# fkluger/vanishing_points_2017

Measured on AMD Instinct MI355X. Metric: images/sec (LSD->CNN->EM) + horizon-AUC parity, YUD-shape, 1/2/4/8 GPU, higher is better.
Workload: dtype f32 (CNN: f32 operands / accumulation / results; conv1 multiply EXACT bf16 pieces of the f32 operands (three per operand) on the bf16 matrix cores; conv2-5, fc6 and fc7 multiply scaled fp16 PAIRS of the f32 operands (22 of 24 significand bits, three exact products per f32 product) on the fp16 matrix

## Files before the change

### __graft_entry__.py

```python
import os
import subprocess
import sys

ROOT = os.path.dirname(os.path.abspath(__file__))
if ROOT not in sys.path:
    sys.path.insert(0, ROOT)


def build():
    from vanishing_points_2017_amd import build as vbuild
    so = vbuild.build(verbose=True)
    sim = os.path.join(ROOT, "tests", "hostsim")
    out = os.path.join(sim, "_build")
    os.makedirs(out, exist_ok=True)
    subprocess.check_call(["g++", "-O2", "-std=c++17", "-ffp-contract=off", "-fPIC", "-shared",
                           "-Wno-unknown-pragmas", os.path.join(sim, "sim_em.cpp"), "-o",
                           os.path.join(out, "libvpk_hostsim.so")])
    subprocess.check_call(["g++", "-O2", "-std=c++17", "-ffp-contract=off", "-fPIC", "-shared",
                           os.path.join(sim, "sim_raster.cpp"), "-o", os.path.join(out, "libvpk_hostsim_raster.so")])
    subprocess.check_call(["g++", "-O2", "-std=c++17", "-Wall", "-Werror", "-fPIC", "-shared",
                           os.path.join(sim, "sim_cnn_plan.cpp"), "-o", os.path.join(out, "libvpk_hostsim_cnn_plan.so")])
    odir = os.path.join(ROOT, "oracle", "_build")
    os.makedirs(odir, exist_ok=True)
    subprocess.check_call(["gcc", "-O2", "-fPIC", "-shared", "-ffp-contract=off", "-fno-builtin",
                           os.path.join(ROOT, "oracle", "_fma.c"), "-o", os.path.join(odir, "libvpkfma.so"), "-lm"])
    import vanishing_points_2017_amd
    from vanishing_points_2017_amd import _lib
    lib = _lib.load()
    missing = [s for s in _lib.EXPORTS if not hasattr(lib, s)]
    if missing:
        raise RuntimeError("libvpk.so lacks symbols: %s" % missing)
    print("built", so)


def smoke():
    import numpy as np
    import torch
    assert torch.cuda.is_available(), "smoke() needs cuda:0"
    from vanishing_points_2017_amd import synth, vp_localisation
    from oracle import em_numpy
    from oracle import agg_raster
    from vanishing_points_2017_amd import sphere_mapping
    sc = synth.make_scene(4242, 90, 3)
    ln = sc["l"]
    sc["sphere_image"] = sphere_mapping.sphere_line_plot(ln.copy(), 500, alpha=0.1)
    assert np.array_equal(sc["sphere_image"], agg_raster.raster(ln)), "the sphere raster differs from the oracle"
    got = vp_localisation.expectation_maximisation(sc["l"].copy(), sc["lp"].copy(), sc["cnn_response"],
                                                   sphere_image=sc["sphere_image"])
    ref = em_numpy.expectation_maximisation(sc["l"].copy(), sc["lp"].copy(), sc["cnn_response"].copy(),
                                            sphere_image=sc["sphere_image"])
    assert np.array_equal(got["vp_assoc"], ref["vp_assoc"]), "line->VP assignments differ from the oracle"
    assert np.abs(got["vp"] - ref["vp"]).max() < 1e-4
    from oracle import cnn_torch
    from vanishing_points_2017_amd import cnn
    w, mean = cnn.synthetic_weights(0), cnn.synthetic_mean(0)
    sphere = sc["sphere_image"][None]
    want = cnn_torch.forward(w, mean, sphere)
    net = cnn.Net(w, mean)
    err = []
    for alg in (4, 2):
        net.set_algorithm(alg)
        err.append(float(np.abs(net.forward(sphere) - want).max()))
    net.set_algorithm(4)
    assert max(err) <= 2e-5, "CNN response differs from the oracle: %s" % err
    print("smoke ok: raster of %d lines exact; %d VPs, %d iterations; CNN max |diff| %.1e (default: fp16 pairs) / %.1e (exact bf16 triples + Winograd f32)" % (
        ln.shape[0], got["vp"].shape[0], got["iterations"], err[0], err[1]))


if __name__ == "__main__":
    build()
    if len(sys.argv) > 1 and sys.argv[1] == "smoke":
        smoke()
```

### vanishing_points_2017_amd/csrc/cnn_dense_pieces.hpp

```cpp
#ifndef VPK_CNN_DENSE_PIECES_HPP_
#define VPK_CNN_DENSE_PIECES_HPP_

namespace {

constexpr int DP_THREADS = 512;
constexpr int DP_BM = 256, DP_BN = 128;
constexpr int DP_CHUNK = 32;
template <int NP> constexpr int DP_STAGE = NP * 2 * 4 * 1024;
constexpr int DP_NST = 3;
constexpr int DP_FOLD = 8;

struct DenseDims {
    int N, K, OC;
    int chunks, kparts, cpp;
    int mtiles, ntiles;
    float wscale, oscale;
    const int* live = nullptr;
};

template <int NP>
__global__ __launch_bounds__(256) void dense_split_kernel(const float* __restrict__ x, unsigned short* __restrict__ out, int N, int K,
                                                          int chunks, float ascale, unsigned* __restrict__ range_word, unsigned range_bit,
                                                          unsigned* __restrict__ img_range, const int* __restrict__ live) {
    const int c = blockIdx.x, nt = blockIdx.y;
    if (live) {
        N = __builtin_amdgcn_readfirstlane(*live);
        if (nt * DP_BN >= N) return;
    }
    const int j = threadIdx.x >> 6, lane = threadIdx.x & 63;
    const int n = nt * DP_BN + 32 * j + (lane & 31), h = lane >> 5;
    float v[16];
    if (n < N) {
        const f32x4v* src = reinterpret_cast<const f32x4v*>(x + (size_t)n * K + (size_t)c * DP_CHUNK + 16 * h);
#pragma unroll
        for (int q = 0; q < 4; ++q) {
            const f32x4v t = src[q];
            v[4 * q] = t[0]; v[4 * q + 1] = t[1]; v[4 * q + 2] = t[2]; v[4 * q + 3] = t[3];
        }
    } else {
#pragma unroll
        for (int e = 0; e < 16; ++e) v[e] = 0.f;
    }
    unsigned short p[3][16];
    bool bad = false;
#pragma unroll
    for (int e = 0; e < 16; ++e) {
        if (NP == 3) split3(v[e], p[0][e], p[1][e], p[2][e]);
        else split2h_guard(v[e] * ascale, p[0][e], p[1][e], bad);
    }
    if (NP == 2) {
        const unsigned long long m = __builtin_amdgcn_ballot_w64(bad);
        if (m != 0ull) {
            if (lane == 0) atomicOr(range_word, range_bit);
            if (img_range && lane < 32 && (((m | (m >> 32)) >> lane) & 1ull)) atomicOr(img_range + n, range_bit);
        }
    }
    u32x4* dst = reinterpret_cast<u32x4*>(out + ((size_t)nt * chunks + c) * (DP_STAGE<NP> / 2));
#pragma unroll
    for (int q = 0; q < NP; ++q)
#pragma unroll
        for (int s = 0; s < 2; ++s) {
            u32x4 w4;
#pragma unroll
            for (int e = 0; e < 4; ++e) w4[e] = (unsigned)p[q][8 * s + 2 * e] | ((unsigned)p[q][8 * s + 2 * e + 1] << 16);
            dst[(((q * 2 + s) * 4 + j) * 64) + lane] = w4;
        }
}

__global__ void dense_tile_weights_kernel(const float* __restrict__ w, float* __restrict__ out, int OC, int K, int chunks, long long total4) {
    const long long o4 = (long long)blockIdx.x * blockDim.x + threadIdx.x;
    if (o4 >= total4) return;
    const int kk4 = (int)(o4 % (DP_CHUNK / 4));
    const int r = (int)((o4 / (DP_CHUNK / 4)) % DP_BM);
    const long long tc = o4 / ((DP_CHUNK / 4) * DP_BM);
    const int c = (int)(tc % chunks);
    const int mt = (int)(tc / chunks);
    const int row = mt * DP_BM + r;
    f32x4v v = {0.f, 0.f, 0.f, 0.f};
    if (row < OC) v = *reinterpret_cast<const f32x4v*>(w + (size_t)row * K + (size_t)c * DP_CHUNK + 4 * kk4);
    reinterpret_cast<f32x4v*>(out)[o4] = v;
}

__global__ void dense_pair_weights_kernel(const float* __restrict__ w, unsigned short* __restrict__ out, int OC, int K, int chunks,
                                          float wscale, long long total16) {
    const long long o = (long long)blockIdx.x * blockDim.x + threadIdx.x;
    if (o >= total16) return;
    const int lane = (int)(o & 63);
    const int q = (int)((o >> 6) & 1), s_ = (int)((o >> 7) & 1), wv = (int)((o >> 8) & 7);
    const long long tc = o >> 11;
    const int c = (int)(tc % chunks), mt = (int)(tc / chunks);
    const int row = mt * DP_BM + 32 * wv + (lane & 31), h = lane >> 5;
    unsigned short p[8];
#pragma unroll
    for (int e = 0; e < 8; ++e) {
        const float x = row < OC ? w[(size_t)row * K + (size_t)c * DP_CHUNK + 16 * h + 8 * s_ + e] * wscale : 0.f;
        unsigned short h0, h1;
        split2h(x, h0, h1);
        p[e] = q == 0 ? h0 : h1;
    }
    u32x4 w4;
#pragma unroll
    for (int e = 0; e < 4; ++e) w4[e] = (unsigned)p[2 * e] | ((unsigned)p[2 * e + 1] << 16);
    reinterpret_cast<u32x4*>(out)[o] = w4;
}

__global__ __launch_bounds__(DP_THREADS, 2) void dense_pairs_kernel(DenseDims d, const unsigned short* __restrict__ wpair,
                                                                    const unsigned short* __restrict__ xfrag, float* __restrict__ part,
                                                                    int* __restrict__ item_counter, int total_items) {
    constexpr int NP = 2;
    __shared__ __attribute__((aligned(16))) unsigned char dp_lds[DP_NST * DP_STAGE<NP>];
    __shared__ int s_next[2];
    const int tid = threadIdx.x, lane = tid & 63;
    const int wave = __builtin_amdgcn_readfirstlane(tid >> 6);
    const int r31 = lane & 31, h = lane >> 5;
    const unsigned lds0 = lds_addr(dp_lds);
    typedef __attribute__((address_space(3))) const bf16x8 lds_cbf8;
    int parity = 0;
    for (int item = blockIdx.x; item < total_items;) {
        int nx = 0;
// ... 227 lines not shown
```

### vanishing_points_2017_amd/csrc/cnn_plan.hpp

```cpp
#ifndef VPK_CNN_PLAN_HPP_
#define VPK_CNN_PLAN_HPP_

#include "../../include/vpk.h"

struct CnnConfig {
    int precision = 0;
    int split_variant = 0;
    int algorithm = 4;
    int fusion = 3;
    int conv1_group = 4;
    int dense_presplit = 1;
    bool profiling = false;
};

inline void cnn_config_set_precision(CnnConfig& c, int mode) {
    c.precision = mode ? 1 : 0;
    c.split_variant = mode > 1 ? mode - 1 : 0;
}

enum class Conv1Impl { GEMM, DIRECT_F32, GEMM_FUSED, PIECES3, PIECES2 };
enum class ConvImpl { DMA_F32, SPLIT_GEMM, WINOGRAD, PIECES3, PIECES2 };
enum class DenseImpl { DMA_F32, PIECES3, PIECES2_STREAMED, PIECES2_PRESPLIT };

struct ConvStage {
    ConvImpl impl = ConvImpl::DMA_F32;
    int split_tiling = 0;
    bool chained_in = false;
    bool chained_out = false;
    bool needs_to_planes = false;
    bool writes_next_planes = false;
};

struct CnnPlan {
    int err = VPK_OK;
    const char* msg = nullptr;
    bool prep_input = false;
    Conv1Impl conv1 = Conv1Impl::PIECES3;
    bool conv1_hands_planes = false;
    ConvStage conv[4];
    bool norm2_planes = false;
    bool norm2_hands_planes = false;
    DenseImpl fc[3] = {DenseImpl::DMA_F32, DenseImpl::DMA_F32, DenseImpl::DMA_F32};
};

inline CnnPlan cnn_resolve_plan(const CnnConfig& c, int tap, bool f32_images, bool device_counted) {
    CnnPlan p;
    const bool f32_mfma = c.precision == 0;
    const bool pairs = f32_mfma && c.algorithm == 4;
    const bool triples = f32_mfma && c.algorithm >= 2 && !pairs;
    const bool wino = f32_mfma && c.algorithm >= 1;
    const bool split = c.precision == 1;

    if (tap == 0 || c.fusion == 0) p.conv1 = Conv1Impl::GEMM;
    else if (c.fusion == 1) p.conv1 = Conv1Impl::DIRECT_F32;
    else if (c.fusion == 2) p.conv1 = Conv1Impl::GEMM_FUSED;
    else p.conv1 = c.fusion == 4 ? Conv1Impl::PIECES2 : Conv1Impl::PIECES3;
    p.prep_input = p.conv1 == Conv1Impl::GEMM || p.conv1 == Conv1Impl::GEMM_FUSED;
    const bool conv1_pieces = p.conv1 == Conv1Impl::PIECES3 || p.conv1 == Conv1Impl::PIECES2;
    p.conv1_hands_planes = conv1_pieces && pairs && tap != 1;
    if (f32_images && p.conv1 == Conv1Impl::PIECES2) {
        p.err = VPK_ERR_STATE;
        p.msg = "vpk_cnn_forward_f32: vpk_cnn_set_fusion(4) takes uint8 rasters only";
    }

    const ConvImpl pieces = pairs ? ConvImpl::PIECES2 : ConvImpl::PIECES3;
    const ConvImpl other = split ? ConvImpl::SPLIT_GEMM : (wino ? ConvImpl::WINOGRAD : ConvImpl::DMA_F32);
    const bool pieces35 = pairs || (triples && c.algorithm == 3);
    p.conv[0].impl = pairs || triples ? pieces : other;
    p.conv[1].impl = pieces35 ? pieces : other;
    p.conv[2].impl = pairs ? pieces : other;
    p.conv[3].impl = pieces35 ? pieces : other;
    p.norm2_planes = pairs;
    p.norm2_hands_planes = pairs && tap != 3;
    p.conv[1].writes_next_planes = pairs && tap != 4;
    p.conv[2].writes_next_planes = pairs && tap != 5;
    p.conv[0].needs_to_planes = (pairs || triples) && !p.conv1_hands_planes;
    p.conv[1].needs_to_planes = pieces35 && !p.norm2_hands_planes;
    p.conv[2].needs_to_planes = pairs && !p.conv[1].writes_next_planes;
    p.conv[3].needs_to_planes = pieces35 && !p.conv[2].writes_next_planes;
    const bool chain = split && tap != 4 && tap != 5;
    p.conv[1].chained_out = p.conv[2].chained_in = p.conv[2].chained_out = p.conv[3].chained_in = chain;
    for (int i = 0; i < 4; ++i) p.conv[i].split_tiling = c.split_variant == 0 ? (i <= 1 ? 1 : 0) : c.split_variant - 1;

    const DenseImpl dense2 = c.dense_presplit ? DenseImpl::PIECES2_PRESPLIT : DenseImpl::PIECES2_STREAMED;
    if (pairs) p.fc[0] = p.fc[1] = dense2;
    else if (triples) p.fc[0] = DenseImpl::PIECES3;

    if (device_counted) {
        const bool counted = p.conv1 == Conv1Impl::PIECES3 && p.conv[0].impl == ConvImpl::PIECES3 &&
                             p.conv[1].impl == ConvImpl::WINOGRAD && p.conv[2].impl == ConvImpl::WINOGRAD &&
                             p.conv[3].impl == ConvImpl::WINOGRAD && !p.norm2_planes && p.fc[0] == DenseImpl::PIECES3 &&
                             p.fc[1] == DenseImpl::DMA_F32 && p.fc[2] == DenseImpl::DMA_F32 && tap < 0 && !c.profiling;
        if (!counted) {
            p.err = VPK_ERR_STATE;
            p.msg = "run_forward: a device-counted pass runs algorithm 2 with the default conv1, untapped";
        }
    }
    return p;
}

#endif
```

### vanishing_points_2017_amd/csrc/cnn_topology.hpp

```cpp
#ifndef VPK_CNN_TOPOLOGY_HPP_
#define VPK_CNN_TOPOLOGY_HPP_

#include <stddef.h>

namespace {

struct Topo { int IC, H, W, OC, OH, OW, G, KH, S, P, BM, OP; };
constexpr Topo TOPO[8] = {
    {1, 500, 500, 96, 123, 123, 1, 11, 4, 0, 96, 0},
    {48, 61, 61, 128, 61, 61, 2, 5, 1, 2, 128, 0},
    {256, 30, 30, 384, 30, 30, 1, 3, 1, 1, 128, 1},
    {192, 30, 30, 192, 30, 30, 2, 3, 1, 1, 96, 1},
    {192, 30, 30, 128, 30, 30, 2, 3, 1, 1, 128, 0},
    {57600, 1, 1, 4096, 1, 1, 1, 1, 1, 0, 128, 0},
    {4096, 1, 1, 4096, 1, 1, 1, 1, 1, 0, 128, 0},
    {4096, 1, 1, 400, 1, 1, 1, 1, 1, 0, 128, 0},
};
constexpr int KSPLIT[8] = {1, 1, 1, 1, 1, 72, 16, 32};
constexpr size_t splitk_partials_per_image() {
    size_t m = 0;
    for (int li = 5; li < 8; ++li) m = (size_t)KSPLIT[li] * TOPO[li].OC > m ? (size_t)KSPLIT[li] * TOPO[li].OC : m;
    return m;
}

enum Region { R_IN, R_CONV1, R_POOL1, R_CONV2, R_POOL2, R_CONV3, R_CONV4, R_CONV5, R_POOL5, R_FCA, R_FCB, R_PART, R_SPLIT, R_SPLIT4, R_SPLIT5, R_P6_2, R_P6_3, R_P6_5, R_COUNT };
constexpr int MAX_CHUNK = 4096;
constexpr size_t CTR_FLOATS = 64;
constexpr size_t GUARD_FLOATS = 64;
static_assert(GUARD_FLOATS * sizeof(float) >= 8 * 16, "the patch DMA's overrun: 8 words of 16 bytes");
constexpr size_t REGION_FLOATS[R_COUNT] = {
    500ull * 500,
    96ull * 123 * 123,
    96ull * 65 * 65,
    256ull * 61 * 61,
    256ull * 32 * 32,
    384ull * 32 * 32,
    384ull * 32 * 32,
    256ull * 900,
    256ull * 225,
    4096, 4096,
    splitk_partials_per_image(),
    96ull * 65 * 65 * 3 / 2,
    384ull * 32 * 32 * 3 / 2,
    384ull * 32 * 32 * 3 / 2,
    96ull * 65 * 65 * 3 / 2,
    256ull * 32 * 32 * 3 / 2,
    384ull * 32 * 32 * 3 / 2,
};
constexpr size_t arena_floats_per_image() {
    size_t t = 0;
    for (int i = 0; i < R_COUNT; ++i) t += REGION_FLOATS[i];
    return t;
}
constexpr size_t A_CONV1 = 96ull * 123 * 123, A_POOL1 = 96ull * 61 * 61;
constexpr size_t A_CONV2 = 256ull * 61 * 61, A_POOL2 = 256ull * 30 * 30;
constexpr size_t A_CONV3 = 384ull * 900, A_CONV4 = 384ull * 900, A_CONV5 = 256ull * 900, A_POOL5 = 256ull * 225;
constexpr size_t A_FC6 = 4096, A_FC7 = 4096, A_FC8 = 400;

}
#endif
```

### vanishing_points_2017_amd/csrc/vpk_cnn.hip

```cpp
#include "vpk_internal.hpp"

#include <stdlib.h>
#include <string.h>
#include <type_traits>
#include <vector>

#include "cnn_plan.hpp"
#include "cnn_topology.hpp"
#include "cnn_gemm_f32.hpp"
#include "cnn_conv1_direct.hpp"
#include "cnn_norm_pool.hpp"

namespace {

#include "cnn_split_gemm.hpp"
#include "cnn_pairs.hpp"
#include "cnn_conv1_pieces.hpp"
#include "cnn_conv_pieces.hpp"
#include "cnn_norm_pool_planes.hpp"
#include "cnn_dense_pieces.hpp"
#include "cnn_winograd.hpp"

struct Layer {
    ConvDims d;
    float* wp = nullptr;
    float* bias = nullptr;
    unsigned* ktab = nullptr;
    unsigned short* wsplit = nullptr;
    float ascale = CP_DEFAULT_ASCALE;
    float hscale = 1.f;
    unsigned short* whalf = nullptr;
    PieceDims pdh;
    SplitDims sd;
    float* wino = nullptr;
    unsigned short* c1frag = nullptr;
    unsigned short* c1half = nullptr;
    float c1scale = 1.f;
    float* c1map = nullptr;
    WinoDims wd;
    Wino5Dims wd5;
    PieceDims pd;
    float* wraw = nullptr;
    unsigned short* wpair = nullptr;
};

}

struct vpk_cnn_state {
    Layer L[8];
    float* mean = nullptr;
    bool loaded = false;
    CnnConfig cfg;
    float* act = nullptr;
    size_t act_bytes = 0;
    int act_batch = 0;
    unsigned short* xfrag = nullptr;
    size_t xfrag_bytes = 0;
    unsigned* range_word = nullptr;
    int range_policy = 0;
    unsigned* img_range = nullptr;
    size_t img_range_bytes = 0;
    int img_range_batch = 0;
    int* rc_list = nullptr;
    unsigned long long* rc_total = nullptr;
    static constexpr int EV_RING = 64;
    hipEvent_t ev[EV_RING][14] = {};
    long long ev_pass = 0;
    bool ev_ready = false;
    bool ev_valid = false;
};

void vpk_cnn_free(vpk_handle* h) {
    if (!h->cnn) return;
    for (auto& l : h->cnn->L) {
        if (l.wp) (void)hipFree(l.wp);
        if (l.bias) (void)hipFree(l.bias);
        if (l.ktab) (void)hipFree(l.ktab);
        if (l.wsplit) (void)hipFree(l.wsplit);
        if (l.whalf) (void)hipFree(l.whalf);
        if (l.wino) (void)hipFree(l.wino);
        if (l.c1frag) (void)hipFree(l.c1frag);
        if (l.c1half) (void)hipFree(l.c1half);
        if (l.c1map) (void)hipFree(l.c1map);
        if (l.wraw) (void)hipFree(l.wraw);
        if (l.wpair) (void)hipFree(l.wpair);
    }
    if (h->cnn->mean) (void)hipFree(h->cnn->mean);
    if (h->cnn->act) (void)hipFree(h->cnn->act);
    if (h->cnn->xfrag) (void)hipFree(h->cnn->xfrag);
    if (h->cnn->range_word) (void)hipFree(h->cnn->range_word);
    if (h->cnn->img_range) (void)hipFree(h->cnn->img_range);
    if (h->cnn->rc_list) (void)hipFree(h->cnn->rc_list);
    if (h->cnn->rc_total) (void)hipFree(h->cnn->rc_total);
    if (h->cnn->ev_ready)
        for (auto& set : h->cnn->ev)
            for (auto& e : set) (void)hipEventDestroy(e);
    delete h->cnn;
    h->cnn = nullptr;
}

namespace {

template <typename KernelT>
void launch_dma(vpk_handle* h, KernelT kernel, const ConvDims& d, int BM, const float* in, const Layer& l, float* out,
                int stride, int* counter, int wpc = 3, const int* live = nullptr) {
    long long ntiles = (d.N + 127) / 128;
    long long total = (long long)d.groups * d.ksplit * ntiles * (d.Mp / BM);
    long long blocks = std::min<long long>(total, (long long)wpc * h->num_cu);
    hipLaunchKernelGGL(kernel, dim3((unsigned)blocks), dim3(CONV_THREADS), 0, h->stream, d, in, l.wp, l.bias, l.ktab,
                       out, stride, counter, (int)total, live);
}

struct FwdCtl {
    unsigned* range_word;
    unsigned* img_range;
    const int* live;
};

struct Images {
    const void* p;
    bool f32;
    const uint8_t* u8() const { return static_cast<const uint8_t*>(p); }
    const float* f() const { return static_cast<const float*>(p); }
    Images at(size_t b) const { return Images{f32 ? (const void*)(f() + b * 250000) : (const void*)(u8() + b * 250000), f32}; }
};

int run_forward(vpk_handle* h, const CnnConfig& cfg, Images img, int batch, float* out, int tap, float* tap_out, const FwdCtl& fc) {
    vpk_cnn_state* S = h->cnn;
    hipStream_t st = h->stream;
    const CnnPlan plan = cnn_resolve_plan(cfg, tap, img.f32, fc.live != nullptr);
    if (plan.err) return vpk_fail(h, plan.err, plan.msg);
    const int* live = fc.live;
    if (batch > S->act_batch) {
        const size_t need = ((size_t)batch * arena_floats_per_image() + GUARD_FLOATS + CTR_FLOATS) * sizeof(float);
        int rc = vpk_reserve(h, (void**)&S->act, &S->act_bytes, need, "hipMalloc(CNN activations)");
        if (rc) return rc;
        VPK_HIP(h, hipMemsetAsync(S->act, 0, need, st));
        S->act_batch = batch;
    }
    float* R[R_COUNT];
    {
        size_t off = 0;
        for (int i = 0; i < R_COUNT; ++i) { R[i] = S->act + off; off += (size_t)S->act_batch * REGION_FLOATS[i]; }
    }
    int* ctr = reinterpret_cast<int*>(S->act + (size_t)S->act_batch * arena_floats_per_image() + GUARD_FLOATS);
    VPK_HIP(h, hipMemsetAsync(ctr, 0, CTR_FLOATS * sizeof(float), st));
    auto tapcopy = [&](int id, const float* src, size_t per) -> int {
        if (tap == id && tap_out)
            VPK_HIP(h, hipMemcpyAsync(tap_out, src, per * batch * sizeof(float), hipMemcpyDeviceToDevice, st));
        return VPK_OK;
    };
    auto ew_blocks = [](long long n) { return (unsigned)((n + 255) / 256); };
    auto tapunpad = [&](int id, const float* src, int C, int H, int W, int pad) {
        if (tap == id && tap_out) {
            const long long planes = (long long)batch * C;
            hipLaunchKernelGGL(unpad_kernel, dim3(ew_blocks(planes * H * W)), dim3(256), 0, st, src, tap_out, planes, H, W,
                               H + 2 * pad, W + 2 * pad, pad);
        }
    };
    auto dims = [&](int li) {
        ConvDims d = S->L[li].d;
        d.B = batch;
        d.N = batch * d.OH * d.OW;
        return d;
    };
    int evi = 0;
    hipEvent_t* evs = S->ev[S->ev_pass % vpk_cnn_state::EV_RING];
    auto mark = [&](int slots) {
        for (; cfg.profiling && slots > 0 && evi < 14; --slots) (void)hipEventRecord(evs[evi++], st);
    };
    int rc;
    mark(1);

    if (plan.prep_input) {
        if (img.f32)
            hipLaunchKernelGGL(prep_input_kernel<float>, dim3((500 * 500 + 255) / 256, batch), dim3(256), 0, st, img.f(), S->mean, R[R_IN],
                               500 * 500);
        else
            hipLaunchKernelGGL(prep_input_kernel<unsigned char>, dim3((500 * 500 + 255) / 256, batch), dim3(256), 0, st, img.u8(), S->mean,
                               R[R_IN], 500 * 500);
    }
    switch (plan.conv1) {
    case Conv1Impl::GEMM:
        launch_dma(h, conv_gemm_dma_kernel<1, 4, 3, 1, false>, dims(0), 96, R[R_IN], S->L[0], R[R_CONV1], 1, ctr + 0);
        mark(1);
        if ((rc = tapcopy(0, R[R_CONV1], A_CONV1))) return rc;
        hipLaunchKernelGGL((lrn5_pool3s2_tiled_kernel<7, 16>), dim3((unsigned)(batch * ((96 + LRN_CCH - 1) / LRN_CCH) * 9 * 4)),
                           dim3(256), 0, st, R[R_CONV1], R[R_POOL1], 96, 123, 123, 61, 61, 1e-4f, 0.75f, 65, 65, 2);
        mark(2);
        break;
    case Conv1Impl::PIECES3:
    case Conv1Impl::PIECES2: {
        const int group = cfg.conv1_group;
        const int total = C1B_PATCHES * ((batch + group - 1) / group);
        unsigned short* c2planes = plan.conv1_hands_planes ? reinterpret_cast<unsigned short*>(R[R_P6_2]) : nullptr;
        if (plan.conv1 == Conv1Impl::PIECES2)
            hipLaunchKernelGGL(conv1_pieces_kernel<2>, dim3((unsigned)std::min(total, h->num_cu)), dim3(C1B_THREADS), 0, st, img.u8(),
                               S->L[0].c1half, S->L[0].c1map, R[R_POOL1], 65, 65, 2, batch, group, 1.f / S->L[0].c1scale, ctr + 0, total,
                               c2planes, S->L[1].ascale, fc.range_word, fc.img_range, live);
// ... 98 lines not shown
                               dst, planes_next, ctr + li, total);
        };
        if (pairs) { if (li == 1) go(conv_pieces_kernel<5, nb, 2, 1>); else if (li == 3) go(conv_pieces_kernel<3, nb, 2, 2>); else go(conv_pieces_kernel<3, nb, 2, 1>); }
        else { if (li == 1) go(conv_pieces_kernel<5, nb, 3, 1>); else go(conv_pieces_kernel<3, nb, 3, 1>); }
    };
    auto conv_stage = [&](int li, const float* src, float* dst, unsigned short* planes, unsigned short* planes_next,
                          const unsigned short* split_in, unsigned short* split_out) {
        const ConvStage& cs = plan.conv[li - 1];
        const bool pairs = cs.impl == ConvImpl::PIECES2;
        switch (cs.impl) {
        case ConvImpl::PIECES3:
        case ConvImpl::PIECES2:
            if (cs.needs_to_planes) to_p6(li, pairs, src, planes);
            conv_pieces(li, pairs, planes, dst, cs.writes_next_planes ? planes_next : nullptr);
            break;
        case ConvImpl::SPLIT_GEMM:
            conv_split(li, cs.split_tiling, src, cs.chained_in ? split_in : nullptr, cs.chained_out ? (void*)split_out : (void*)dst, cs.chained_out);
            break;
        case ConvImpl::WINOGRAD:
            conv_wino(li, src, dst);
            break;
        case ConvImpl::DMA_F32:
            if (li == 3) launch_dma(h, conv_gemm_dma_kernel<1, 4, 3, 1, false>, dims(3), 96, src, S->L[3], dst, 1, ctr + 3);
            else launch_dma(h, conv_gemm_dma_kernel<2, 2, 2, 2, false>, dims(li), 128, src, S->L[li], dst, 1, ctr + li);
            break;
        }
    };
    unsigned short* p6_2 = reinterpret_cast<unsigned short*>(R[R_P6_2]);
    unsigned short* p6_3 = reinterpret_cast<unsigned short*>(R[R_P6_3]);
    unsigned short* p6_5 = reinterpret_cast<unsigned short*>(R[R_P6_5]);
    unsigned short* s4 = reinterpret_cast<unsigned short*>(R[R_SPLIT4]);
    unsigned short* s5 = reinterpret_cast<unsigned short*>(R[R_SPLIT5]);
    conv_stage(1, R[R_POOL1], R[R_CONV2], p6_2, nullptr, nullptr, nullptr);
    mark(1);
    if ((rc = tapcopy(2, R[R_CONV2], A_CONV2))) return rc;
    if (plan.norm2_planes)
        hipLaunchKernelGGL((lrn5_pool3s2_planes_kernel<6>), dim3((unsigned)(batch * 5 * 8)), dim3(256), 0, st, R[R_CONV2], R[R_POOL2],
                           plan.norm2_hands_planes ? p6_3 : nullptr, 256, 61, 61, 30, 30, 1e-4f, 32, 32, 1, 8,
                           S->L[2].ascale, fc.range_word, 1u << 2, fc.img_range);
    else
        hipLaunchKernelGGL((lrn5_pool3s2_stream_kernel<6, 4>), dim3((unsigned)(batch * 5 * 8)), dim3(256), 0, st, R[R_CONV2], R[R_POOL2],
                           256, 61, 61, 30, 30, 1e-4f, 0.75f, 32, 32, 1, 8, live);
    mark(2);
    tapunpad(3, R[R_POOL2], 256, 30, 30, 1);
    conv_stage(2, R[R_POOL2], R[R_CONV3], p6_3, p6_5, nullptr, s4);
    mark(1);
    tapunpad(4, R[R_CONV3], 384, 30, 30, 1);
    conv_stage(3, R[R_CONV3], R[R_CONV4], p6_5, p6_3, s4, s5);
    mark(1);
    tapunpad(5, R[R_CONV4], 384, 30, 30, 1);
    conv_stage(4, R[R_CONV4], R[R_CONV5], plan.conv[2].writes_next_planes ? p6_3 : p6_5, nullptr, s5, nullptr);
    mark(1);
    if ((rc = tapcopy(6, R[R_CONV5], A_CONV5))) return rc;
    hipLaunchKernelGGL((pool5_kernel<8>), dim3((unsigned)(((long long)batch * 256 + 7) / 8)), dim3(256), 0, st, R[R_CONV5], R[R_POOL5],
                       (long long)batch * 256, live);
    mark(1);
    if ((rc = tapcopy(7, R[R_POOL5], A_POOL5))) return rc;

    float* fc_in = R[R_POOL5];
    float* fc_out = R[R_FCA];
    for (int li = 5; li < 8; ++li) {
        ConvDims d = dims(li);
        const DenseImpl impl = plan.fc[li - 5];
        if (impl == DenseImpl::DMA_F32) {
            launch_dma(h, conv_gemm_dma_kernel<2, 2, 2, 2, true>, d, 128, fc_in, S->L[li], R[R_PART], 1, ctr + li, 3, live);
        } else {
            const bool pairs = impl != DenseImpl::PIECES3;
            DenseDims dd;
            dd.N = batch; dd.K = d.K; dd.OC = d.OC; dd.chunks = d.K / DP_CHUNK;
            dd.kparts = li == 5 ? 45 : 16;
            dd.cpp = dd.chunks / dd.kparts;
            dd.mtiles = (d.OC + DP_BM - 1) / DP_BM; dd.ntiles = (batch + DP_BN - 1) / DP_BN;
            dd.wscale = pairs ? S->L[li].hscale : 1.f;
            dd.live = live;
            dd.oscale = pairs ? 1.f / (S->L[li].hscale * S->L[li].ascale) : 1.f;
            const size_t need = (size_t)dd.ntiles * (TOPO[5].IC / DP_CHUNK) * DP_STAGE<3>;
            if ((rc = vpk_reserve(h, (void**)&S->xfrag, &S->xfrag_bytes, need, "hipMalloc(dense input fragments)"))) return rc;
            const int total = dd.mtiles * dd.ntiles * dd.kparts;
            const dim3 split_grid((unsigned)dd.chunks, (unsigned)dd.ntiles), grid((unsigned)std::min(total, h->num_cu));
            if (pairs)
                hipLaunchKernelGGL(dense_split_kernel<2>, split_grid, dim3(256), 0, st, fc_in, S->xfrag, batch,
                                   d.K, dd.chunks, S->L[li].ascale, fc.range_word, 1u << li, fc.img_range, nullptr);
            else
                hipLaunchKernelGGL(dense_split_kernel<3>, split_grid, dim3(256), 0, st, fc_in, S->xfrag, batch,
                                   d.K, dd.chunks, 1.f, fc.range_word, 0u, nullptr, live);
            switch (impl) {
            case DenseImpl::PIECES2_PRESPLIT:
                hipLaunchKernelGGL(dense_pairs_kernel, grid, dim3(DP_THREADS), 0, st, dd, S->L[li].wpair, S->xfrag, R[R_PART], ctr + li, total);
                break;
            case DenseImpl::PIECES2_STREAMED:
                hipLaunchKernelGGL(dense_pieces_kernel<2>, grid, dim3(DP_THREADS), 0, st, dd, S->L[li].wraw, S->xfrag, R[R_PART], ctr + li, total);
                break;
            default:
                hipLaunchKernelGGL(dense_pieces_kernel<3>, grid, dim3(DP_THREADS), 0, st, dd, S->L[li].wraw, S->xfrag, R[R_PART], ctr + li, total);
                break;
            }
            d.ksplit = dd.kparts;
        }
        const long long tot = (long long)d.N * d.OC;
        float* dst = li == 7 ? out : fc_out;
        float* pre = (li == 7 && tap == 10) ? tap_out : nullptr;
        hipLaunchKernelGGL(splitk_reduce_kernel, dim3(ew_blocks(tot)), dim3(256), 0, st, R[R_PART], S->L[li].bias, d.ksplit,
                           d.N, d.OC, li == 7 ? 2 : 1, dst, pre, live);
        mark(1);
        if (li == 5 && (rc = tapcopy(8, fc_out, A_FC6))) return rc;
        if (li == 6 && (rc = tapcopy(9, fc_out, A_FC7))) return rc;
        fc_in = fc_out;
        fc_out = (li == 5) ? R[R_FCB] : R[R_FCA];
    }
    if (cfg.profiling) {
        S->ev_valid = (evi == 14);
        if (S->ev_valid) ++S->ev_pass;
    }
    VPK_HIP(h, hipGetLastError());
    return VPK_OK;
}

}
#include "cnn_calibrate.hpp"
#include "cnn_range_policy.hpp"

namespace {

struct ScopedDeviceBuffer {
    void* p = nullptr;
    ~ScopedDeviceBuffer() { if (p) (void)hipFree(p); }
};

template <typename T>
int upload(vpk_handle* h, T** dst, const T* src, size_t n) {
    VPK_HIP(h, hipMalloc((void**)dst, n * sizeof(T)));
    VPK_HIP(h, hipMemcpy(*dst, src, n * sizeof(T), hipMemcpyHostToDevice));
    return VPK_OK;
}

int load_model(vpk_handle* h, const float* const blobs[16], const float* mean) {
    vpk_cnn_state* S = h->cnn;
    int rc;
    if ((rc = upload(h, &S->mean, mean, (size_t)500 * 500))) return rc;
    if (const char* e = getenv("VPK_CONV1_GROUP")) { const int v = atoi(e); if (v >= 1 && v <= 64) S->cfg.conv1_group = v; }
    if (const char* e = getenv("VPK_DENSE_PRESPLIT")) S->cfg.dense_presplit = atoi(e) != 0;
    for (int li = 0; li < 8; ++li) {
        const Topo& t = TOPO[li];
        const float* w = blobs[2 * li];
        Layer& l = S->L[li];
        ConvDims& d = l.d;
        d.B = 0; d.IC = t.IC; d.Hp = t.H + 2 * t.P; d.Wp = t.W + 2 * t.P; d.OC = t.OC; d.OH = t.OH; d.OW = t.OW; d.groups = t.G;
        d.OHp = t.OH + 2 * t.OP; d.OWp = t.OW + 2 * t.OP; d.opad = t.OP;
        if (li == 0) { d.IC = C1_PH * C1_PH; d.Hp = C1_PW; d.Wp = C1_PW; }
        d.K = t.IC * t.KH * t.KH;
        d.Kp = (d.K + BK - 1) / BK * BK;
        d.Mp = (t.OC + t.BM - 1) / t.BM * t.BM;
        d.N = 0;
        d.ksplit = KSPLIT[li];
        d.relu = 1;
        const size_t w_floats = (size_t)t.G * t.OC * d.K;
        const size_t p_floats = (size_t)t.G * d.Kp * d.Mp;
        {
            ScopedDeviceBuffer rawbuf;
            VPK_HIP(h, hipMalloc(&rawbuf.p, w_floats * sizeof(float)));
            const float* raw = static_cast<const float*>(rawbuf.p);
            VPK_HIP(h, hipMemcpy(rawbuf.p, w, w_floats * sizeof(float), hipMemcpyHostToDevice));
            VPK_HIP(h, hipMalloc((void**)&l.wp, p_floats * sizeof(float)));
            hipLaunchKernelGGL(pack_weights_kernel, dim3((unsigned)((p_floats + 255) / 256)), dim3(256), 0, h->stream, raw,
                               l.wp, t.G, t.OC, d.K, d.Kp, d.Mp);
            VPK_HIP(h, hipStreamSynchronize(h->stream));
            if (li == 5 || li == 6) {
                const int chunks = d.K / DP_CHUNK, mtiles = (t.OC + DP_BM - 1) / DP_BM;
                const long long total4 = (long long)mtiles * chunks * DP_BM * (DP_CHUNK / 4);
                VPK_HIP(h, hipMalloc((void**)&l.wraw, (size_t)total4 * 16));
                hipLaunchKernelGGL(dense_tile_weights_kernel, dim3((unsigned)((total4 + 255) / 256)), dim3(256), 0, h->stream, raw, l.wraw, t.OC, d.K,
                                   chunks, total4);
                VPK_HIP(h, hipStreamSynchronize(h->stream));
                l.hscale = weight_scale_pow2(w, w_floats);
                const long long total16 = (long long)mtiles * chunks * 8 * 2 * 2 * 64;
                VPK_HIP(h, hipMalloc((void**)&l.wpair, (size_t)total16 * 16));
                hipLaunchKernelGGL(dense_pair_weights_kernel, dim3((unsigned)((total16 + 255) / 256)), dim3(256), 0, h->stream, raw, l.wpair, t.OC,
                                   d.K, chunks, l.hscale, total16);
                VPK_HIP(h, hipStreamSynchronize(h->stream));
            }
        }
        if (li < 5) {
            std::vector<unsigned> tab(d.Kp, 0u);
            for (int k = 0; k < d.K; ++k) {
                int ic = k / (t.KH * t.KH), r = k % (t.KH * t.KH), kh = r / t.KH, kw = r % t.KH;
                if (li == 0)
                    tab[k] = (unsigned)((((kh % C1_PH) * C1_PH + kw % C1_PH) * C1_PW + kh / C1_PH) * C1_PW + kw / C1_PH) * 4u;
                else
                    tab[k] = (unsigned)((ic * d.Hp + kh) * d.Wp + kw) * 4u;
            }
            if ((rc = upload(h, &l.ktab, tab.data(), tab.size()))) return rc;
        }
        if (li >= 1 && li <= 4) {
            SplitDims& sd = l.sd;
// ... 159 lines not shown
    for (int i = 0; i < CAL_N; ++i) scales[i] = h->cnn->L[CAL_LAYER[i]].ascale;
    return VPK_OK;
}

int vpk_cnn_set_activation_scales(vpk_handle* h, const float scales[6]) {
    if (!h || !scales) return vpk_fail(h, VPK_ERR_ARG, "vpk_cnn_set_activation_scales: null argument");
    if (!h->cnn || !h->cnn->loaded) return vpk_fail(h, VPK_ERR_STATE, "vpk_cnn_set_activation_scales before vpk_cnn_load");
    for (int i = 0; i < CAL_N; ++i) {
        int ex = 0;
        const float f = std::frexp(scales[i], &ex);
        if (!(scales[i] > 0.f) || !std::isfinite(scales[i]) || f != 0.5f || ex < -99 || ex > 101)
            return vpk_fail(h, VPK_ERR_ARG, "vpk_cnn_set_activation_scales: every scale must be a power of two in 2^-100 .. 2^100");
    }
    for (int i = 0; i < CAL_N; ++i) h->cnn->L[CAL_LAYER[i]].ascale = scales[i];
    return VPK_OK;
}

int vpk_cnn_range_flags(vpk_handle* h, uint32_t* flags_out) {
    if (!h) return VPK_ERR_ARG;
    if (!h->cnn || !h->cnn->loaded) return vpk_fail(h, VPK_ERR_STATE, "vpk_cnn_range_flags before vpk_cnn_load");
    VPK_HIP(h, hipSetDevice(h->device));
    unsigned word = 0;
    VPK_HIP(h, hipMemcpyAsync(&word, h->cnn->range_word, sizeof(word), hipMemcpyDeviceToHost, h->stream));
    VPK_HIP(h, hipMemsetAsync(h->cnn->range_word, 0, sizeof(word), h->stream));
    VPK_HIP(h, hipStreamSynchronize(h->stream));
    if (flags_out) *flags_out = word;
    if (!word) return VPK_OK;
    static const char* names[8] = {"", "conv2", "conv3", "conv4", "conv5", "fc6", "fc7", ""};
    std::string msg = "vpk_cnn_forward: scaled fp16-pair activations reached fp16's range (clamped to 65504) at the input of";
    for (int li = 1; li <= 6; ++li)
        if (word & (1u << li)) msg += std::string(" ") + names[li];
    msg += ": the response maps of the forwards since the last check are NOT the net's; recalibrate (vpk_cnn_calibrate) or use vpk_cnn_set_algorithm(2)";
    return vpk_fail(h, VPK_ERR_RANGE, msg.c_str());
}

}

namespace {
int forward_chunks(vpk_handle* h, Images sphere, int batch, float* out, int tap, float* tap_out, bool policy) {
    if (!h || !sphere.p || !out || batch < 1) return vpk_fail(h, VPK_ERR_ARG, "vpk_cnn_forward: bad argument");
    if (!sphere.f32 && ((size_t)sphere.p & 3) != 0)
        return vpk_fail(h, VPK_ERR_ARG, "vpk_cnn_forward: the rasters must be 4-byte aligned");
    if (sphere.f32 && ((size_t)sphere.p & 15) != 0)
        return vpk_fail(h, VPK_ERR_ARG, "vpk_cnn_forward_f32: the images must be 16-byte aligned");
    if (!h->cnn || !h->cnn->loaded) return vpk_fail(h, VPK_ERR_STATE, "vpk_cnn_forward before vpk_cnn_load");
    VPK_HIP(h, hipSetDevice(h->device));
    const size_t per_img = arena_floats_per_image() * sizeof(float);
    int chunk = (int)std::min<size_t>(std::min<size_t>((size_t)batch, MAX_CHUNK),
                                      std::max<size_t>(1, (h->total_mem / 3) / per_img));
    static const size_t tap_size[11] = {A_CONV1, A_POOL1, A_CONV2, A_POOL2, A_CONV3, A_CONV4, A_CONV5, A_POOL5,
                                        A_FC6, A_FC7, A_FC8};
    vpk_cnn_state* S = h->cnn;
    if (policy) {
        int rc = vpk_reserve(h, (void**)&S->img_range, &S->img_range_bytes, (size_t)batch * sizeof(unsigned), "hipMalloc(per-image range flags)");
        if (rc) return rc;
        VPK_HIP(h, hipMemsetAsync(S->img_range, 0, (size_t)batch * sizeof(unsigned), h->stream));
        S->img_range_batch = batch;
    }
    const bool recompute = policy && S->range_policy == 1 && S->cfg.precision == 0 && S->cfg.algorithm == 4;
    for (int b0 = 0; b0 < batch; b0 += chunk) {
        int nb = std::min(chunk, batch - b0);
        float* tp = (tap_out && tap >= 0 && tap <= 10) ? tap_out + (size_t)b0 * tap_size[tap] : nullptr;
        const Images sp = sphere.at((size_t)b0);
        float* op = out + (size_t)b0 * 400;
        unsigned* img = policy ? S->img_range + b0 : nullptr;
        int rc = run_forward(h, S->cfg, sp, nb, op, tp ? tap : -1, tp, FwdCtl{recompute ? S->range_word + 1 : S->range_word, img, nullptr});
        if (!rc && recompute) rc = recompute_flagged(h, sp, nb, op, img);
        if (rc) return rc;
    }
    return VPK_OK;
}
}

extern "C" {

int vpk_cnn_forward_tap(vpk_handle* h, const uint8_t* sphere, int batch, float* out, int tap, float* tap_out) {
    return forward_chunks(h, Images{sphere, false}, batch, out, tap, tap_out, false);
}

int vpk_cnn_forward(vpk_handle* h, const uint8_t* sphere, int batch, float* out) {
    return forward_chunks(h, Images{sphere, false}, batch, out, -1, nullptr, true);
}

int vpk_cnn_forward_tap_f32(vpk_handle* h, const float* image, int batch, float* out, int tap, float* tap_out) {
    return forward_chunks(h, Images{image, true}, batch, out, tap, tap_out, false);
}

int vpk_cnn_forward_f32(vpk_handle* h, const float* image, int batch, float* out) {
    return forward_chunks(h, Images{image, true}, batch, out, -1, nullptr, true);
}

int vpk_cnn_set_range_policy(vpk_handle* h, int policy) {
    if (!h || !h->cnn) return vpk_fail(h, VPK_ERR_STATE, "vpk_cnn_set_range_policy before vpk_cnn_load");
    if (policy != 0 && policy != 1) return vpk_fail(h, VPK_ERR_ARG, "vpk_cnn_set_range_policy: policy must be 0 (RAISE) or 1 (RECOMPUTE_EXACT)");
    h->cnn->range_policy = policy;
    return VPK_OK;
}

int vpk_cnn_image_range_flags(vpk_handle* h, int batch, uint32_t* flags_out) {
    if (!h || !flags_out || batch < 1) return vpk_fail(h, VPK_ERR_ARG, "vpk_cnn_image_range_flags: bad argument");
    if (!h->cnn || !h->cnn->loaded) return vpk_fail(h, VPK_ERR_STATE, "vpk_cnn_image_range_flags before vpk_cnn_load");
    if (h->cnn->img_range_batch == 0) return vpk_fail(h, VPK_ERR_STATE, "vpk_cnn_image_range_flags before any vpk_cnn_forward");
    if (batch != h->cnn->img_range_batch)
        return vpk_fail(h, VPK_ERR_ARG, "vpk_cnn_image_range_flags: batch differs from the last vpk_cnn_forward's");
    VPK_HIP(h, hipSetDevice(h->device));
    VPK_HIP(h, hipMemcpyAsync(flags_out, h->cnn->img_range, (size_t)batch * sizeof(uint32_t), hipMemcpyDeviceToHost, h->stream));
    VPK_HIP(h, hipStreamSynchronize(h->stream));
    return VPK_OK;
}

int vpk_cnn_recomputed(vpk_handle* h, int64_t* n_out) {
    if (!h || !n_out) return vpk_fail(h, VPK_ERR_ARG, "vpk_cnn_recomputed: null argument");
    if (!h->cnn || !h->cnn->loaded) return vpk_fail(h, VPK_ERR_STATE, "vpk_cnn_recomputed before vpk_cnn_load");
    VPK_HIP(h, hipSetDevice(h->device));
    unsigned long long n = 0;
    VPK_HIP(h, hipMemcpyAsync(&n, h->cnn->rc_total, sizeof(n), hipMemcpyDeviceToHost, h->stream));
    VPK_HIP(h, hipMemsetAsync(h->cnn->rc_total, 0, sizeof(n), h->stream));
    VPK_HIP(h, hipStreamSynchronize(h->stream));
    *n_out = (int64_t)n;
// ... 5 lines not shown
```

Baseline: 22600.

## Fuse pool5 and fc6 reduce with fp16-pair splitting into dense input fragments

Adds a pool5 kernel that max-pools in shared memory and writes fc6's fp16-pair input fragments directly. It also adds a fc6 split-k reduce kernel that applies bias and ReLU and emits fc7's fragments, so the separate dense_split passes and their f32 activation round-trips are skipped. The counter and per-image range-flag memsets are merged into one control block cleared by a single memset. Both fused paths are disabled when a tap needs the intermediate f32 tensor, and the fragment layout and range reporting must match the original split kernel exactly.

New measurement: 22650, median of 2. Within noise of the previous version (+0.2%).

```diff
diff --git a/__graft_entry__.py b/__graft_entry__.py
--- a/__graft_entry__.py
+++ b/__graft_entry__.py
@@ -20,6 +20,8 @@
                            os.path.join(sim, "sim_raster.cpp"), "-o", os.path.join(out, "libvpk_hostsim_raster.so")])
     subprocess.check_call(["g++", "-O2", "-std=c++17", "-Wall", "-Werror", "-fPIC", "-shared",
                            os.path.join(sim, "sim_cnn_plan.cpp"), "-o", os.path.join(out, "libvpk_hostsim_cnn_plan.so")])
+    subprocess.check_call(["g++", "-O2", "-std=c++17", "-Wall", "-Werror", "-fPIC", "-shared",
+                           os.path.join(sim, "sim_cnn_plan_glue.cpp"), "-o", os.path.join(out, "libvpk_hostsim_cnn_plan_glue.so")])
     odir = os.path.join(ROOT, "oracle", "_build")
     os.makedirs(odir, exist_ok=True)
     subprocess.check_call(["gcc", "-O2", "-fPIC", "-shared", "-ffp-contract=off", "-fno-builtin",
diff --git a/vanishing_points_2017_amd/csrc/cnn_dense_pieces.hpp b/vanishing_points_2017_amd/csrc/cnn_dense_pieces.hpp
--- a/vanishing_points_2017_amd/csrc/cnn_dense_pieces.hpp
+++ b/vanishing_points_2017_amd/csrc/cnn_dense_pieces.hpp
@@ -65,6 +65,116 @@
             for (int e = 0; e < 4; ++e) w4[e] = (unsigned)p[q][8 * s + 2 * e] | ((unsigned)p[q][8 * s + 2 * e + 1] << 16);
             dst[(((q * 2 + s) * 4 + j) * 64) + lane] = w4;
         }
+}
+
+constexpr int DP_WORDS = DP_STAGE<2> / 16;
+
+template <int PL>
+__global__ __launch_bounds__(256) void pool5_split_kernel(const float* __restrict__ in, unsigned short* __restrict__ out, int N, int chunks,
+                                                          float ascale, unsigned* __restrict__ range_word, unsigned range_bit,
+                                                          unsigned* __restrict__ img_range) {
+    constexpr int H = 30, W = 30, P = 15, HW = H * W, PP = P * P, G = 256 / PL, NW = PL * PP / 8;
+    static_assert(256 % PL == 0 && (PL * PP) % 8 == 0 && NW <= 256, "whole words per workgroup, one thread per word");
+    __shared__ __attribute__((aligned(16))) float s[PL * HW];
+    __shared__ __attribute__((aligned(16))) float pooled[PL * PP];
+    const int n = blockIdx.x / G, g = blockIdx.x % G;
+    const int t = threadIdx.x;
+    bool bad = false;
+    u32x4 w0 = {0u, 0u, 0u, 0u}, w1 = {0u, 0u, 0u, 0u};
+    if (n < N) {
+        const f32x4v* src = reinterpret_cast<const f32x4v*>(in + ((size_t)n * 256 + (size_t)g * PL) * HW);
+        for (int q = t; q < PL * HW / 4; q += 256) reinterpret_cast<f32x4v*>(s)[q] = src[q];
+        __syncthreads();
+        for (int e = t; e < PL * PP; e += 256) {
+            const int pl = e / PP, o = e - pl * PP;
+            const int py = o / P, px = o - py * P;
+            const float* x = s + pl * HW + (2 * py) * W + 2 * px;
+            const bool by = 2 * py + 2 < H, bx = 2 * px + 2 < W;
+            float m = fmaxf(fmaxf(x[0], x[1]), fmaxf(x[W], x[W + 1]));
+            if (bx) m = fmaxf(m, fmaxf(x[2], x[W + 2]));
+            if (by) m = fmaxf(m, fmaxf(x[2 * W], x[2 * W + 1]));
+            if (bx && by) m = fmaxf(m, x[2 * W + 2]);
+            pooled[e] = m;
+        }
+        __syncthreads();
+        if (t < NW) {
+            const f32x4v a = reinterpret_cast<const f32x4v*>(pooled)[2 * t], b = reinterpret_cast<const f32x4v*>(pooled)[2 * t + 1];
+            const float v[8] = {a[0], a[1], a[2], a[3], b[0], b[1], b[2], b[3]};
+            unsigned short p0[8], p1[8];
+#pragma unroll
+            for (int e = 0; e < 8; ++e) split2h_guard(v[e] * ascale, p0[e], p1[e], bad);
+#pragma unroll
+            for (int e = 0; e < 4; ++e) {
+                w0[e] = (unsigned)p0[2 * e] | ((unsigned)p0[2 * e + 1] << 16);
+                w1[e] = (unsigned)p1[2 * e] | ((unsigned)p1[2 * e + 1] << 16);
+            }
+        }
+        range_report(bad, range_word, range_bit, img_range ? img_range + n : nullptr);
+    }
+    if (t < NW) {
+        const int k = g * (PL * PP) + 8 * t;
+        const int c = k >> 5, h = (k >> 4) & 1, sp = (k >> 3) & 1;
+        const int nt = n / DP_BN, j = (n % DP_BN) >> 5, lane = (n & 31) + 32 * h;
+        u32x4* dst = reinterpret_cast<u32x4*>(out) + ((size_t)nt * chunks + c) * DP_WORDS + (sp * 4 + j) * 64 + lane;
+        dst[0] = w0;
+        dst[2 * 4 * 64] = w1;
+    }
+}
+
+__global__ __launch_bounds__(256) void reduce_split_kernel(const float* __restrict__ part, const float* __restrict__ bias, int ksplit, int N,
+                                                           int OC, unsigned short* __restrict__ out, int chunks, float ascale,
+                                                           unsigned* __restrict__ range_word, unsigned range_bit,
+                                                           unsigned* __restrict__ img_range) {
+    __shared__ float sums[32][DP_CHUNK + 1];
+    const int c = blockIdx.x, j = blockIdx.y & 3, nt = blockIdx.y >> 2;
+    const int t = threadIdx.x;
+    const int n0 = nt * DP_BN + 32 * j;
+    if (n0 < N) {
+        const int r = t >> 3, m4 = t & 7, n = n0 + r;
+        f32x4v v = {0.f, 0.f, 0.f, 0.f};
+        if (n < N) {
+            const float* src = part + (size_t)n * OC + (size_t)c * DP_CHUNK + 4 * m4;
+            const size_t step = (size_t)N * OC;
+#pragma unroll 9
+            for (int sk = 0; sk < ksplit; ++sk) {
+                const f32x4v p = *reinterpret_cast<const f32x4v*>(src + sk * step);
+                v[0] += p[0]; v[1] += p[1]; v[2] += p[2]; v[3] += p[3];
+            }
+            const f32x4v bv = *reinterpret_cast<const f32x4v*>(bias + c * DP_CHUNK + 4 * m4);
+#pragma unroll
+            for (int e = 0; e < 4; ++e) {
+                v[e] += bv[e];
+                v[e] = v[e] > 0.f ? v[e] : 0.f;
+            }
+        }
+#pragma unroll
+        for (int e = 0; e < 4; ++e) sums[r][4 * m4 + e] = v[e];
+        __syncthreads();
+    }
+    if (t < 128) {
+        const int lane = t & 63, sp = t >> 6, h = lane >> 5, n = n0 + (lane & 31);
+        bool bad = false;
+        unsigned short p0[8], p1[8];
+#pragma unroll
+        for (int e = 0; e < 8; ++e) {
+            const float x = n0 < N ? sums[lane & 31][16 * h + 8 * sp + e] : 0.f;
+            split2h_guard(x * ascale, p0[e], p1[e], bad);
+        }
+        const unsigned long long m = __builtin_amdgcn_ballot_w64(bad);
+        if (m != 0ull) {
+            if (lane == 0) atomicOr(range_word, range_bit);
+            if (img_range && lane < 32 && (((m | (m >> 32)) >> lane) & 1ull)) atomicOr(img_range + n, range_bit);
+        }
+        u32x4 w0, w1;
+#pragma unroll
+        for (int e = 0; e < 4; ++e) {
+            w0[e] = (unsigned)p0[2 * e] | ((unsigned)p0[2 * e + 1] << 16);
+            w1[e] = (unsigned)p1[2 * e] | ((unsigned)p1[2 * e + 1] << 16);
+        }
+        u32x4* dst = reinterpret_cast<u32x4*>(out) + ((size_t)nt * chunks + c) * DP_WORDS + (sp * 4 + j) * 64 + lane;
+        dst[0] = w0;
+        dst[2 * 4 * 64] = w1;
+    }
 }
 
 __global__ void dense_tile_weights_kernel(const float* __restrict__ w, float* __restrict__ out, int OC, int K, int chunks, long long total4) {
diff --git a/vanishing_points_2017_amd/csrc/cnn_plan.hpp b/vanishing_points_2017_amd/csrc/cnn_plan.hpp
--- a/vanishing_points_2017_amd/csrc/cnn_plan.hpp
+++ b/vanishing_points_2017_amd/csrc/cnn_plan.hpp
@@ -10,6 +10,7 @@
     int fusion = 3;
     int conv1_group = 4;
     int dense_presplit = 1;
+    int fc_glue = 1;
     bool profiling = false;
 };
 
@@ -40,6 +41,8 @@
     ConvStage conv[4];
     bool norm2_planes = false;
     bool norm2_hands_planes = false;
+    bool pool5_splits = false;
+    bool fc6_reduce_splits = false;
     DenseImpl fc[3] = {DenseImpl::DMA_F32, DenseImpl::DMA_F32, DenseImpl::DMA_F32};
 };
 
@@ -85,12 +88,15 @@
     const DenseImpl dense2 = c.dense_presplit ? DenseImpl::PIECES2_PRESPLIT : DenseImpl::PIECES2_STREAMED;
     if (pairs) p.fc[0] = p.fc[1] = dense2;
     else if (triples) p.fc[0] = DenseImpl::PIECES3;
+    p.pool5_splits = pairs && c.fc_glue != 0 && tap != 7;
+    p.fc6_reduce_splits = pairs && c.fc_glue != 0 && tap != 8;
 
     if (device_counted) {
         const bool counted = p.conv1 == Conv1Impl::PIECES3 && p.conv[0].impl == ConvImpl::PIECES3 &&
                              p.conv[1].impl == ConvImpl::WINOGRAD && p.conv[2].impl == ConvImpl::WINOGRAD &&
                              p.conv[3].impl == ConvImpl::WINOGRAD && !p.norm2_planes && p.fc[0] == DenseImpl::PIECES3 &&
-                             p.fc[1] == DenseImpl::DMA_F32 && p.fc[2] == DenseImpl::DMA_F32 && tap < 0 && !c.profiling;
+                             p.fc[1] == DenseImpl::DMA_F32 && p.fc[2] == DenseImpl::DMA_F32 && !p.pool5_splits &&
+                             !p.fc6_reduce_splits && tap < 0 && !c.profiling;
         if (!counted) {
             p.err = VPK_ERR_STATE;
             p.msg = "run_forward: a device-counted pass runs algorithm 2 with the default conv1, untapped";
diff --git a/vanishing_points_2017_amd/csrc/cnn_topology.hpp b/vanishing_points_2017_amd/csrc/cnn_topology.hpp
--- a/vanishing_points_2017_amd/csrc/cnn_topology.hpp
+++ b/vanishing_points_2017_amd/csrc/cnn_topology.hpp
@@ -25,7 +25,7 @@
 
 enum Region { R_IN, R_CONV1, R_POOL1, R_CONV2, R_POOL2, R_CONV3, R_CONV4, R_CONV5, R_POOL5, R_FCA, R_FCB, R_PART, R_SPLIT, R_SPLIT4, R_SPLIT5, R_P6_2, R_P6_3, R_P6_5, R_COUNT };
 constexpr int MAX_CHUNK = 4096;
-constexpr size_t CTR_FLOATS = 64;
+constexpr size_t CTR_WORDS = 64;
 constexpr size_t GUARD_FLOATS = 64;
 static_assert(GUARD_FLOATS * sizeof(float) >= 8 * 16, "the patch DMA's overrun: 8 words of 16 bytes");
 constexpr size_t REGION_FLOATS[R_COUNT] = {
diff --git a/vanishing_points_2017_amd/csrc/vpk_cnn.hip b/vanishing_points_2017_amd/csrc/vpk_cnn.hip
--- a/vanishing_points_2017_amd/csrc/vpk_cnn.hip
+++ b/vanishing_points_2017_amd/csrc/vpk_cnn.hip
@@ -58,8 +58,9 @@
     size_t xfrag_bytes = 0;
     unsigned* range_word = nullptr;
     int range_policy = 0;
+    unsigned* ctl = nullptr;
+    size_t ctl_bytes = 0;
     unsigned* img_range = nullptr;
-    size_t img_range_bytes = 0;
     int img_range_batch = 0;
     int* rc_list = nullptr;
     unsigned long long* rc_total = nullptr;
@@ -89,7 +90,7 @@
     if (h->cnn->act) (void)hipFree(h->cnn->act);
     if (h->cnn->xfrag) (void)hipFree(h->cnn->xfrag);
     if (h->cnn->range_word) (void)hipFree(h->cnn->range_word);
-    if (h->cnn->img_range) (void)hipFree(h->cnn->img_range);
+    if (h->cnn->ctl) (void)hipFree(h->cnn->ctl);
     if (h->cnn->rc_list) (void)hipFree(h->cnn->rc_list);
     if (h->cnn->rc_total) (void)hipFree(h->cnn->rc_total);
     if (h->cnn->ev_ready)
@@ -115,7 +116,18 @@
     unsigned* range_word;
     unsigned* img_range;
     const int* live;
+    int clear_images = 0;
 };
+
+constexpr size_t ctl_image_words(size_t images) { return (images + 31) / 32 * 32; }
+static_assert(CTR_WORDS % 32 == 0, "the counters are whole 128-byte lines too");
+
+int reserve_ctl(vpk_handle* h, size_t images) {
+    vpk_cnn_state* S = h->cnn;
+    const int rc = vpk_reserve(h, (void**)&S->ctl, &S->ctl_bytes, (CTR_WORDS + ctl_image_words(images)) * sizeof(unsigned), "hipMalloc(CNN control block)");
+    S->img_range = rc ? nullptr : S->ctl + CTR_WORDS;
+    return rc;
+}
 
 struct Images {
     const void* p;
@@ -132,7 +144,7 @@
     if (plan.err) return vpk_fail(h, plan.err, plan.msg);
     const int* live = fc.live;
     if (batch > S->act_batch) {
-        const size_t need = ((size_t)batch * arena_floats_per_image() + GUARD_FLOATS + CTR_FLOATS) * sizeof(float);
+        const size_t need = ((size_t)batch * arena_floats_per_image() + GUARD_FLOATS) * sizeof(float);
         int rc = vpk_reserve(h, (void**)&S->act, &S->act_bytes, need, "hipMalloc(CNN activations)");
         if (rc) return rc;
         VPK_HIP(h, hipMemsetAsync(S->act, 0, need, st));
@@ -143,8 +155,8 @@
         size_t off = 0;
         for (int i = 0; i < R_COUNT; ++i) { R[i] = S->act + off; off += (size_t)S->act_batch * REGION_FLOATS[i]; }
     }
-    int* ctr = reinterpret_cast<int*>(S->act + (size_t)S->act_batch * arena_floats_per_image() + GUARD_FLOATS);
-    VPK_HIP(h, hipMemsetAsync(ctr, 0, CTR_FLOATS * sizeof(float), st));
+    int* ctr = reinterpret_cast<int*>(S->ctl);
+    VPK_HIP(h, hipMemsetAsync(ctr, 0, (CTR_WORDS + ctl_image_words((size_t)fc.clear_images)) * sizeof(unsigned), st));
     auto tapcopy = [&](int id, const float* src, size_t per) -> int {
         if (tap == id && tap_out)
             VPK_HIP(h, hipMemcpyAsync(tap_out, src, per * batch * sizeof(float), hipMemcpyDeviceToDevice, st));
@@ -349,8 +361,17 @@
     conv_stage(4, R[R_CONV4], R[R_CONV5], plan.conv[2].writes_next_planes ? p6_3 : p6_5, nullptr, s5, nullptr);
     mark(1);
     if ((rc = tapcopy(6, R[R_CONV5], A_CONV5))) return rc;
-    hipLaunchKernelGGL((pool5_kernel<8>), dim3((unsigned)(((long long)batch * 256 + 7) / 8)), dim3(256), 0, st, R[R_CONV5], R[R_POOL5],
-                       (long long)batch * 256, live);
+    const int dense_ntiles = (batch + DP_BN - 1) / DP_BN;
+    if (plan.fc[0] != DenseImpl::DMA_F32 &&
+        (rc = vpk_reserve(h, (void**)&S->xfrag, &S->xfrag_bytes, (size_t)dense_ntiles * (TOPO[5].IC / DP_CHUNK) * DP_STAGE<3>,
+                          "hipMalloc(dense input fragments)")))
+        return rc;
+    if (plan.pool5_splits)
+        hipLaunchKernelGGL((pool5_split_kernel<8>), dim3((unsigned)(dense_ntiles * DP_BN * (256 / 8))), dim3(256), 0, st, R[R_CONV5], S->xfrag,
+                           batch, TOPO[5].IC / DP_CHUNK, S->L[5].ascale, fc.range_word, 1u << 5, fc.img_range);
+    else
+        hipLaunchKernelGGL((pool5_kernel<8>), dim3((unsigned)(((long long)batch * 256 + 7) / 8)), dim3(256), 0, st, R[R_CONV5], R[R_POOL5],
+                           (long long)batch * 256, live);
     mark(1);
     if ((rc = tapcopy(7, R[R_POOL5], A_POOL5))) return rc;
 
@@ -367,18 +388,17 @@
             dd.N = batch; dd.K = d.K; dd.OC = d.OC; dd.chunks = d.K / DP_CHUNK;
             dd.kparts = li == 5 ? 45 : 16;
             dd.cpp = dd.chunks / dd.kparts;
-            dd.mtiles = (d.OC + DP_BM - 1) / DP_BM; dd.ntiles = (batch + DP_BN - 1) / DP_BN;
+            dd.mtiles = (d.OC + DP_BM - 1) / DP_BM; dd.ntiles = dense_ntiles;
             dd.wscale = pairs ? S->L[li].hscale : 1.f;
             dd.live = live;
             dd.oscale = pairs ? 1.f / (S->L[li].hscale * S->L[li].ascale) : 1.f;
-            const size_t need = (size_t)dd.ntiles * (TOPO[5].IC / DP_CHUNK) * DP_STAGE<3>;
-            if ((rc = vpk_reserve(h, (void**)&S->xfrag, &S->xfrag_bytes, need, "hipMalloc(dense input fragments)"))) return rc;
             const int total = dd.mtiles * dd.ntiles * dd.kparts;
             const dim3 split_grid((unsigned)dd.chunks, (unsigned)dd.ntiles), grid((unsigned)std::min(total, h->num_cu));
-            if (pairs)
+            const bool have_frags = li == 5 ? plan.pool5_splits : plan.fc6_reduce_splits;
+            if (!have_frags && pairs)
                 hipLaunchKernelGGL(dense_split_kernel<2>, split_grid, dim3(256), 0, st, fc_in, S->xfrag, batch,
                                    d.K, dd.chunks, S->L[li].ascale, fc.range_word, 1u << li, fc.img_range, nullptr);
-            else
+            else if (!have_frags)
                 hipLaunchKernelGGL(dense_split_kernel<3>, split_grid, dim3(256), 0, st, fc_in, S->xfrag, batch,
                                    d.K, dd.chunks, 1.f, fc.range_word, 0u, nullptr, live);
             switch (impl) {
@@ -397,8 +417,13 @@
         const long long tot = (long long)d.N * d.OC;
         float* dst = li == 7 ? out : fc_out;
         float* pre = (li == 7 && tap == 10) ? tap_out : nullptr;
-        hipLaunchKernelGGL(splitk_reduce_kernel, dim3(ew_blocks(tot)), dim3(256), 0, st, R[R_PART], S->L[li].bias, d.ksplit,
-                           d.N, d.OC, li == 7 ? 2 : 1, dst, pre, live);
+        if (li == 5 && plan.fc6_reduce_splits)
+            hipLaunchKernelGGL(reduce_split_kernel, dim3((unsigned)(TOPO[6].IC / DP_CHUNK), (unsigned)(4 * dense_ntiles)), dim3(256), 0, st,
+                               R[R_PART], S->L[5].bias, d.ksplit, batch, d.OC, S->xfrag, TOPO[6].IC / DP_CHUNK, S->L[6].ascale,
+                               fc.range_word, 1u << 6, fc.img_range);
+        else
+            hipLaunchKernelGGL(splitk_reduce_kernel, dim3(ew_blocks(tot)), dim3(256), 0, st, R[R_PART], S->L[li].bias, d.ksplit,
+                               d.N, d.OC, li == 7 ? 2 : 1, dst, pre, live);
         mark(1);
         if (li == 5 && (rc = tapcopy(8, fc_out, A_FC6))) return rc;
         if (li == 6 && (rc = tapcopy(9, fc_out, A_FC7))) return rc;
@@ -437,6 +462,8 @@
     if ((rc = upload(h, &S->mean, mean, (size_t)500 * 500))) return rc;
     if (const char* e = getenv("VPK_CONV1_GROUP")) { const int v = atoi(e); if (v >= 1 && v <= 64) S->cfg.conv1_group = v; }
     if (const char* e = getenv("VPK_DENSE_PRESPLIT")) S->cfg.dense_presplit = atoi(e) != 0;
+    if (const char* e = getenv("VPK_FC_GLUE")) S->cfg.fc_glue = atoi(e) != 0;
+    if ((rc = reserve_ctl(h, MAX_CHUNK))) return rc;
     for (int li = 0; li < 8; ++li) {
         const Topo& t = TOPO[li];
         const float* w = blobs[2 * li];
@@ -702,9 +729,8 @@
                                         A_FC6, A_FC7, A_FC8};
     vpk_cnn_state* S = h->cnn;
     if (policy) {
-        int rc = vpk_reserve(h, (void**)&S->img_range, &S->img_range_bytes, (size_t)batch * sizeof(unsigned), "hipMalloc(per-image range flags)");
+        int rc = reserve_ctl(h, (size_t)batch);
         if (rc) return rc;
-        VPK_HIP(h, hipMemsetAsync(S->img_range, 0, (size_t)batch * sizeof(unsigned), h->stream));
         S->img_range_batch = batch;
     }
     const bool recompute = policy && S->range_policy == 1 && S->cfg.precision == 0 && S->cfg.algorithm == 4;
@@ -714,7 +740,8 @@
         const Images sp = sphere.at((size_t)b0);
         float* op = out + (size_t)b0 * 400;
         unsigned* img = policy ? S->img_range + b0 : nullptr;
-        int rc = run_forward(h, S->cfg, sp, nb, op, tp ? tap : -1, tp, FwdCtl{recompute ? S->range_word + 1 : S->range_word, img, nullptr});
+        int rc = run_forward(h, S->cfg, sp, nb, op, tp ? tap : -1, tp,
+                             FwdCtl{recompute ? S->range_word + 1 : S->range_word, img, nullptr, policy && b0 == 0 ? batch : 0});
         if (!rc && recompute) rc = recompute_flagged(h, sp, nb, op, img);
         if (rc) return rc;
     }
```
